# jeffersonfparil/poolgen

Hardware: NVIDIA B200
Metric: loci/sec for ols_iter (f64) (higher is better)
Workload: dtype f64

## Files before the change

poolgen_b200/csrc/pg_api.cu:

```cuda
#include <math.h>
#include <stdarg.h>
#include <stdio.h>
#include <stdlib.h>
#include <string.h>

#include <algorithm>
#include <new>

#include "pg_internal.h"
#include "pg_ptable.h"

namespace pg {
cudaError_t launch_scan_a2(const ScanParams &, int, cudaStream_t);
cudaError_t launch_scan_a3(const ScanParams &, int, cudaStream_t);
cudaError_t launch_scan_a4(const ScanParams &, int, cudaStream_t);
cudaError_t launch_scan_a5(const ScanParams &, int, cudaStream_t);
cudaError_t launch_scan_a6(const ScanParams &, int, cudaStream_t);

cudaError_t launch_scan(const ScanParams &p, int sm_count, cudaStream_t s) {
    switch (p.lay.A) {
        case 2: return launch_scan_a2(p, sm_count, s);
        case 3: return launch_scan_a3(p, sm_count, s);
        case 4: return launch_scan_a4(p, sm_count, s);
        case 5: return launch_scan_a5(p, sm_count, s);
// ... 460 lines not shown
        int rc = text_stage_a(b, b->text_src, b->text_bytes, (size_t)at + 1);
        if (rc) return rc;
        L = pg::text_parse_finish(&b->text, b->stream, &ce, &at);
    }
    if (L < 0) return pg::text_parse_fail(ctx, "upload_sync_text", L, ce, at, s->n, b->cap);
    b->n_loci = L;
    if (n_loci_out) *n_loci_out = L;
    if (L > 0 && is_regression(s))
        PG_CUDA(ctx, pg::launch_ingest_u32((const uint32_t *)b->d_stage.get(), L, s->n, s->A_in, s->drop_col, s->lay,
                                           ingest_out(b, 0), b->stream));
    return PG_OK;
}

int pg_batch_upload_sync_text(pg_batch *b, const char *text, size_t n_bytes, int64_t *n_loci_out) {
    if (n_loci_out) *n_loci_out = 0;
    int rc = text_stage_a(b, text, n_bytes, 0);
    if (rc) return rc;
    rc = text_stage_b(b, n_loci_out);
    if (rc) return rc;
    PG_CUDA(b->scan->ctx, cudaStreamSynchronize(b->stream));
    return PG_OK;
}

int pg_batch_text_labels(pg_batch *b, const uint64_t **line_offsets, const uint64_t **positions) {
    if (!b) return PG_ERR_ARG;
    if (!b->text.parsed) return fail(b->scan->ctx, PG_ERR_STATE, "pg_batch_text_labels before pg_batch_upload_sync_text");
    if (line_offsets) *line_offsets = b->text.h_out_offset.get();
    if (positions) *positions = b->text.h_out_pos.get();
    return PG_OK;
}

int pg_batch_synth(pg_batch *b, uint64_t seed, int64_t first_locus, int64_t n_loci) {
    if (!b) return PG_ERR_ARG;
    pg_scan *s = b->scan;
    pg_ctx *ctx = s->ctx;
    if (n_loci < 0 || n_loci > b->cap) return fail(ctx, PG_ERR_ARG, "synth: %lld loci > capacity %lld", (long long)n_loci, (long long)b->cap);
    PG_CUDA(ctx, cudaSetDevice(ctx->device));
    b->n_loci = n_loci;
    b->have_input = 1;
    if (n_loci == 0) return PG_OK;
    const size_t per_locus = (size_t)s->A_in * s->n * 4;
    if (!is_regression(s)) {
        int rc = ensure_stage(b, (size_t)b->cap * per_locus);
        if (rc) return rc;
        PG_CUDA(ctx, pg::launch_synth(seed, first_locus, n_loci, s->n, s->A_in, (uint32_t *)b->d_stage.get(), b->stream));
        b->input_is_counts = 1;
        return PG_OK;
    }
    int64_t slice = (int64_t)((size_t)256 << 20) / (int64_t)per_locus;
    if (slice < 1) slice = 1;
    if (slice > n_loci) slice = n_loci;
    if (b->d_stage.capacity() < (size_t)slice * per_locus) {
        int rc = ensure_stage(b, (size_t)slice * per_locus);
        if (rc) return rc;
    } else {
        slice = (int64_t)(b->d_stage.capacity() / per_locus);
        if (slice > n_loci) slice = n_loci;
    }
    for (int64_t l0 = 0; l0 < n_loci; l0 += slice) {
        const int64_t m = (n_loci - l0 < slice) ? n_loci - l0 : slice;
        PG_CUDA(ctx, pg::launch_synth(seed, first_locus + l0, m, s->n, s->A_in, (uint32_t *)b->d_stage.get(), b->stream));
        PG_CUDA(ctx, pg::launch_ingest_u32((const uint32_t *)b->d_stage.get(), m, s->n, s->A_in, s->drop_col, s->lay,
                                           ingest_out(b, l0), b->stream));
    }
    b->input_is_counts = 1;
    return PG_OK;
}

static int run_once(pg_batch *b, int *launches) {
    pg_scan *s = b->scan;
    pg_ctx *ctx = s->ctx;
    if (!b->have_input) return fail(ctx, PG_ERR_STATE, "pg_batch_run: no input uploaded");
    if (b->n_loci == 0) return PG_OK;
    if (is_regression(s)) {
        int kpass = pg::max_phen_per_pass(s->A_dev);
        {
            const int fit = (int)((size_t)(96 * 1024) / ((size_t)s->lay.n_pad * 8)) - (s->weighted ? 1 : 0);
            if (kpass > fit) kpass = fit < 1 ? 1 : fit;
        }
        static const int nbuf_env = getenv("PG_NBUF") ? atoi(getenv("PG_NBUF")) : 0;
        static const int warps_env = getenv("PG_WARPS") ? atoi(getenv("PG_WARPS")) : 0;
        static const int g_env = getenv("PG_G") ? atoi(getenv("PG_G")) : 0;
        static const int p_env = getenv("PG_P") ? atoi(getenv("PG_P")) : 0;
        if (is_nm(s)) kpass = 1;
        for (int base = 0; base < (is_nm(s) ? 1 : s->k); base += kpass) {
            pg::ScanParams p;
            memset(&p, 0, sizeof p);
            p.lay = s->lay;
            p.freq = b->d_freq.get();
            p.depth = b->d_depth.get();
            p.dmin = b->d_dmin.get();
            p.hint = b->d_hint.get();
            p.n_loci = b->n_loci;
            p.kind = is_nm(s) ? PG_KIND_OLS : s->kind;
            p.filter_only = is_nm(s) ? 1 : 0;
            p.weighted = s->weighted;
            p.maf = s->maf;
            p.one_minus_maf = 1.00 - s->maf;
            p.max_miss = s->max_miss;
            p.min_depth_f = (double)s->min_depth;
            p.w_uniform = s->w_uniform;
            p.df = s->df;
            p.inv_df = 1.0 / s->df;
            p.inv_n = 1.0 / (double)s->n;
            p.inv_nm2 = 1.0 / ((double)s->n - 2.0);
            p.ln_beta = s->ln_beta;
            p.ptab = s->d_ptab.get();
            p.ptab_isd = s->ptab_isd;
            p.ptab_bits = s->ptab_bits;
            p.ptab_t1 = s->ptab_t1;
            p.ptab_t0 = s->ptab_t0;
            p.ptab_M = s->ptab_M;
            p.K = std::min(kpass, s->k - base);
            p.y_has_nan = s->y_has_nan;
            p.yc = s->d_yc.get() + (size_t)base * s->lay.n_pad;
            p.w = s->d_w.get();
            for (int j = 0; j < p.K; j++) {
                p.ysum[j] = s->ysum[base + j];
                p.syy[j] = s->syy[base + j];
                p.ymean[j] = s->ymean[base + j];
            }
            for (int j = 0; j < s->A_dev; j++) p.codes[j] = s->codes_dev[j];
            p.meta = b->d_meta.get();
            p.freq_mean = b->d_fmean.get();
            p.stats = b->d_stats.get();
            p.defer_list = b->d_defer.get();
            p.defer_count = reinterpret_cast<uint32_t *>(b->d_defer.get() + b->cap);
            p.k_total = s->k;
            p.phen_base = base;
            p.write_meta = base == 0;
            p.nbuf_override = nbuf_env;
            p.warps_override = warps_env;
            p.g_override = g_env;
            p.p_override = p_env;
            PG_CUDA(ctx, pg::launch_scan(p, ctx->sm_count, b->stream));
            if (launches) (*launches) += 2;
        }
        if (is_nm(s)) {
            pg::NmParams q;
            memset(&q, 0, sizeof q);
            q.lay = s->lay;
            q.freq = b->d_freq.get();
            q.depth = b->d_depth.get();
            q.n_loci = b->n_loci;
            q.kind = s->kind;
            q.k = s->k;
            q.yraw = s->d_yraw.get();
            q.gw_sig = s->gw_sig;
            q.gw_min = s->gw_min;
            q.gw_max = s->gw_max;
            q.df = s->df;
            q.ln_beta = s->ln_beta;
            q.ptab = s->d_ptab.get();
            q.ptab_isd = s->ptab_isd;
            q.ptab_bits = s->ptab_bits;
            q.ptab_t1 = s->ptab_t1;
            q.ptab_t0 = s->ptab_t0;
            q.ptab_M = s->ptab_M;
            for (int j = 0; j < s->A_dev; j++) q.codes[j] = s->codes_dev[j];
            q.meta = b->d_meta.get();
            q.stats = b->d_stats.get();
            PG_CUDA(ctx, pg::launch_nm(q, ctx->sm_count, b->stream));
            if (launches) (*launches)++;
        }
    } else {
        pg::TableParams p;
        memset(&p, 0, sizeof p);
        p.counts = (const uint32_t *)b->d_stage.get();
        p.n_loci = b->n_loci;
        p.n = s->n;
        p.A_in = s->A_in;
        p.kind = s->kind;
        p.drop_col = s->drop_col;
        p.maf = s->maf;
        p.one_minus_maf = 1.00 - s->maf;
        p.max_miss = s->max_miss;
        p.min_depth_f = (double)s->min_depth;
        p.w = s->d_w.get();
// ... 187 lines not shown
```

poolgen_b200/csrc/pg_ingest.cu:

```cuda
#include <stdlib.h>

#include "pg_device.cuh"
#include "pg_internal.h"

namespace pg {

struct HintParams {
    double maf, one_minus_maf, min_depth_f;
    int enabled;
};
__device__ __forceinline__ unsigned ambiguous_alleles(const double *q, int A, int n, const HintParams &hp) {
    const double tol_rel = 4.0 * ((double)n + 8.0) * kEps;
    unsigned amb = 0;
    for (int j = 0; j < A; j++) {
        const double tl = tol_rel * fmax(fabs(q[j]), 1.0);
        if (fabs(q[j] - hp.maf) <= tl || fabs(q[j] - hp.one_minus_maf) <= tl) amb |= 1u << j;
    }
    return amb;
}

__device__ __forceinline__ uint8_t locus_hint(const double *q, int A, int n, uint32_t dm, const HintParams &hp,
                                              unsigned exact) {
    if (!hp.enabled) return 0;
    const double tol_rel = 4.0 * ((double)n + 8.0) * kEps;
    unsigned kept = 0;
    bool removed_with_reads = false, safe = true;
    for (int j = 0; j < A; j++) {
        const double tl = tol_rel * fmax(fabs(q[j]), 1.0);
        if (!((exact >> j) & 1u) && (fabs(q[j] - hp.maf) <= tl || fabs(q[j] - hp.one_minus_maf) <= tl)) safe = false;
        if (!((q[j] < hp.maf) | (q[j] > hp.one_minus_maf)))
            kept |= 1u << j;
        else if (q[j] > 0.0)
            removed_with_reads = true;
    }
    const bool depth_ok = dm != 0u && !((double)dm < hp.min_depth_f);
    return (safe && depth_ok && removed_with_reads && __popc(kept) >= 2) ? (uint8_t)(0x80u | kept) : (uint8_t)0;
}

template <typename RowFn>
__device__ __forceinline__ void ingest_loci(int64_t n_loci, const Layout &lay, int P, const double *freq,
                                            const double *__restrict__ w, uint32_t *__restrict__ dmin,
                                            uint8_t *__restrict__ hint, const HintParams &hp, RowFn &&row) {
    const int lane = threadIdx.x & 31, sub = lane / P, q0 = lane % P, lpw = 32 / P;
    const int64_t gw = ((int64_t)blockIdx.x * blockDim.x + threadIdx.x) >> 5;
    const int64_t nw = ((int64_t)gridDim.x * blockDim.x) >> 5;
    for (int64_t l0 = gw * lpw; l0 < n_loci; l0 += nw * lpw) {
        const int64_t locus = l0 + sub;
        double q[PG_MAX_ALLELES] = {0, 0, 0, 0, 0, 0};
        uint32_t dm = 0xFFFFFFFFu;
        if (locus < n_loci)
            for (int i = q0; i < lay.n_pad; i += P) row(locus, i, q, dm);
        for (int off = P >> 1; off >= 1; off >>= 1) {
            for (int j = 0; j < lay.A; j++) q[j] += __shfl_xor_sync(0xFFFFFFFFu, q[j], off);
            dm = min(dm, __shfl_xor_sync(0xFFFFFFFFu, dm, off));
        }
        unsigned amb = (hp.enabled && locus < n_loci && dm != 0u) ? ambiguous_alleles(q, lay.A, lay.n, hp) : 0u;
        if (__any_sync(0xFFFFFFFFu, amb != 0u)) {
            __syncwarp();
            const double *fl = freq + (size_t)(locus < n_loci ? locus : 0) * lay.freq_stride();
            for (int j = 0; j < lay.A; j++) {
                if (!__any_sync(0xFFFFFFFFu, (amb >> j) & 1u)) continue;
                double e = 0.0;
                for (int r0 = 0; r0 < lay.n; r0 += P) {
                    const int i = r0 + q0;
                    double term = 0.0;
                    if (i < lay.n && locus < n_loci) {
                        const double f = __ldcg(fl + lay.freq_off(i, j));
                        term = (f != f) ? 0.0 : __dmul_rn(f, w[i]);
                    }
                    const int m = min(P, lay.n - r0);
                    for (int t = 0; t < m; t++) e = __dadd_rn(e, __shfl_sync(0xFFFFFFFFu, term, t, P));
                }
                if ((amb >> j) & 1u) q[j] = e;
            }
        }
        if (locus < n_loci && q0 == 0) {
            dmin[locus] = dm;
            hint[locus] = locus_hint(q, lay.A, lay.n, dm, hp, amb);
        }
    }
}

template <typename CT>
__global__ void __launch_bounds__(256) ingest_counts_kernel(const CT *__restrict__ counts, int64_t n_loci, int n,
                                                            int A_in, int drop_col, Layout lay, int P,
                                                            double *__restrict__ freq, uint32_t *__restrict__ depth,
                                                            uint32_t *__restrict__ dmin, uint8_t *__restrict__ hint,
                                                            const double *__restrict__ w, HintParams hp) {
    ingest_loci(n_loci, lay, P, freq, w, dmin, hint, hp, [&](int64_t locus, int i, double *q, uint32_t &dm) {
        double *fl = freq + (size_t)locus * lay.freq_stride();
        if (i >= n) {
            for (int j = 0; j < lay.A; j++) fl[lay.freq_off(i, j)] = 0.0;
            depth[(size_t)locus * lay.n_pad + i] = 0xFFFFFFFFu;
            return;
        }
        const CT *cl = counts + (size_t)locus * A_in * n + i;
        uint32_t c[PG_MAX_ALLELES];
        uint64_t d = 0;
        int jj = 0;
        for (int j = 0; j < A_in; j++) {
            if (j == drop_col) continue;
            c[jj] = (uint32_t)cl[(size_t)j * n];
            d += c[jj];
            jj++;
        }
        if (d > 0xFFFFFFFEull) d = 0xFFFFFFFEull;
        const double dd = (double)d, wi = w[i];
        const double rd = __drcp_rn(dd);
        for (int j = 0; j < lay.A; j++) {
            const double cj = (double)c[j];
            const double q0 = __dmul_rn(cj, rd);
            const double f = (d == 0) ? nan("") : __fma_rn(__fma_rn(-q0, dd, cj), rd, q0);
            fl[lay.freq_off(i, j)] = f;
            if (d != 0) q[j] = fma(f, wi, q[j]);
        }
        depth[(size_t)locus * lay.n_pad + i] = (uint32_t)d;
        dm = min(dm, (uint32_t)d);
    });
}
// ... 106 lines not shown
```

poolgen_b200/csrc/pg_internal.h:

```cpp
#pragma once
#include <cuda_runtime.h>
#include <stdint.h>
#include <string>
#include <utility>
#include <vector>

#include "poolgen_cuda.h"
#include "pg_synth.h"

namespace pg {

__host__ __device__ constexpr int chunk_rows(int A) { return A <= 2 ? 256 : (A == 3 ? 192 : 128); }

struct Layout {
    int n;
    int n_pad;
    int A;
    int rc;
    int n_chunks;
    int rc_last;
    __host__ __device__ size_t freq_stride() const { return (size_t)A * n_pad; }
    __host__ __device__ size_t depth_stride() const { return (size_t)n_pad; }
    __host__ __device__ size_t freq_off(int i, int j) const {
        int c = i / rc, r = i - c * rc;
        int rcc = (c == n_chunks - 1) ? rc_last : rc;
        return (size_t)c * A * rc + (size_t)j * rcc + r;
    }
};

inline Layout make_layout(int n, int A) {
    Layout l;
    l.n = n;
    l.n_pad = (n + 3) & ~3;
    l.A = A;
    const int cr = chunk_rows(A);
    if (l.n_pad <= cr) {
        l.rc = l.n_pad;
        l.n_chunks = 1;
        l.rc_last = l.n_pad;
    } else {
        l.rc = cr;
        l.n_chunks = (l.n_pad + cr - 1) / cr;
        l.rc_last = l.n_pad - (l.n_chunks - 1) * cr;
    }
    return l;
}

constexpr int kMaxPhenPerPass = 4;
inline int max_phen_per_pass(int A) { return A <= 4 ? 4 : (A == 5 ? 3 : 2); }

struct ScanParams {
    Layout lay;
    const double *freq;
    const uint32_t *depth;
    const uint32_t *dmin;
    const uint8_t *hint;
    int64_t n_loci;
    int kind;
    int weighted;
    double maf, one_minus_maf, max_miss;
    double min_depth_f;
    double w_uniform;
    double df;
    double inv_df;
    double inv_n, inv_nm2;
    double ln_beta;
    const void *ptab;
    double ptab_isd, ptab_bits, ptab_t1, ptab_t0;
    int ptab_M;
    const double *yc;
    const double *w;
    double ysum[kMaxPhenPerPass];
    double syy[kMaxPhenPerPass];
    double ymean[kMaxPhenPerPass];
    int y_has_nan;
    int filter_only;
    uint8_t codes[8];
    uint64_t *meta;
    double *freq_mean;
    double *stats;
    uint64_t *defer_list;
    uint32_t *defer_count;
    int k_total, phen_base, K;
    int write_meta;
    uint32_t common_bytes, warp_bytes, stage_bytes;
    int nbuf, block_loci;
    int nbuf_override, warps_override, g_override, p_override;
};

struct TableParams {
    const uint32_t *counts;
    int64_t n_loci;
    int n, A_in;
    int kind;
    int drop_col;
    double maf, one_minus_maf, max_miss, min_depth_f;
    const double *w;
    uint8_t codes[8];
    uint64_t *meta;
    double *stats;
};

struct NmParams {
    Layout lay;
    const double *freq;
    const uint32_t *depth;
    int64_t n_loci;
    int kind;
    int k;
    const double *yraw;
    double gw_sig, gw_min, gw_max;
    double df, ln_beta;
    const void *ptab;
    double ptab_isd, ptab_bits, ptab_t1, ptab_t0;
    int ptab_M;
    uint8_t codes[8];
    uint64_t *meta;
    double *stats;
};
cudaError_t launch_nm(const NmParams &p, int sm_count, cudaStream_t s);

constexpr int kKinMleMaxM = 13;
struct KinMleParams {
    const double *G;
    int64_t P;
    int n, ldg, m, k;
    const double *Z;
    const double *fix;
    double df, ln_beta;
    const void *ptab;
    double ptab_isd, ptab_bits, ptab_t1, ptab_t0;
    int ptab_M;
    double *beta, *var, *pval;
};
cudaError_t launch_kin_mle(const KinMleParams &p, int sm_count, cudaStream_t s);

cudaError_t launch_scan(const ScanParams &p, int sm_count, cudaStream_t s);
cudaError_t launch_tables(const TableParams &p, int sm_count, cudaStream_t s);
struct IngestOut {
    double *freq;
    uint32_t *depth;
    uint32_t *dmin;
    uint8_t *hint;
    const double *w;
    double maf, one_minus_maf, min_depth_f;
};
cudaError_t launch_ingest_u32(const uint32_t *counts, int64_t n_loci, int n, int A_in, int drop_col, const Layout &lay,
                              const IngestOut &o, cudaStream_t s);
cudaError_t launch_ingest_u16(const uint16_t *counts, int64_t n_loci, int n, int A_in, int drop_col, const Layout &lay,
                              const IngestOut &o, cudaStream_t s);
cudaError_t launch_ingest_u8(const uint8_t *counts, int64_t n_loci, int n, int A_in, int drop_col, const Layout &lay,
                             const IngestOut &o, cudaStream_t s);
cudaError_t launch_ingest_freq(const double *freq_in, const uint32_t *depth_in, int64_t n_loci, int n, const Layout &lay,
                               const IngestOut &o, cudaStream_t s);
cudaError_t launch_synth(uint64_t seed, int64_t first_locus, int64_t n_loci, int n, int A_in,
                         uint32_t *counts, cudaStream_t s);
cudaError_t launch_widen(const void *src, int elem_bytes, uint32_t *dst, size_t count, cudaStream_t s);

template <typename T, bool Pinned>
// ... 154 lines not shown
```

poolgen_b200/csrc/pg_scan.cuh:

```cuda
#pragma once
#include "pg_device.cuh"
#include "pg_internal.h"

namespace pg {

constexpr int kScanWarps = 12;
constexpr int kRedPitch = 33;

template <int A, int K, bool W>
struct Acc {
    static constexpr int S0 = 0;
    static constexpr int P0 = S0 + A;
    static constexpr int C0 = P0 + A * (A + 1) / 2;
    static constexpr int Q0 = C0 + A * K;
    static constexpr int N = Q0 + (W ? A : 0);
    static constexpr int NP = N | 1;
    __host__ __device__ static constexpr int tri(int j, int l) {
        return P0 + j * A - j * (j - 1) / 2 + (l - j);
    }
};

template <int A, int K, bool W, bool NANAWARE>
__device__ __forceinline__ void accum_row(double (&acc)[Acc<A, K, W>::N], const double (&f)[A], const double (&y)[K],
                                          double w) {
// ... 973 lines not shown
    for (int k = 0; k < K; k++) {
        const double ptrue = in[k] ? exp(fma(s[k], fma(s[k], fma(s[k], c23[k].y, c23[k].x), c01[k].y), c01[k].x)) : 0.0;
        const double ib = 0.5 * ptrue;
        const double cdf = t_abs[k] <= tab.t_one ? 0.5 : 1.0 - ib;
        if (need[k]) pv[k] = 2.0 * (1.0 - cdf);
    }
}

template <int A, int K, int KIND>
__device__ __noinline__ void write_records(const ScanParams &p, const PTableDev &tab, int64_t locus, int status,
                                           int m, unsigned cb, const double *tb) {
    constexpr int T2 = 2 * (A - 1) * K;
    if (p.write_meta) {
        uint64_t mv = (uint64_t)status;
        if (status == PG_LOCUS_OK) {
            mv |= (uint64_t)m << 8;
#pragma unroll
            for (int s = 0; s < A - 1; s++)
                if (s < m) mv |= (uint64_t)p.codes[slot_col(cb, s)] << (16 + 8 * s);
            if (kind_is_ols<KIND>(p) && m < 6) mv |= (uint64_t)p.codes[(cb >> 20) & 0xfu] << (16 + 8 * m);
        }
        p.meta[locus] = mv;
#pragma unroll
        for (int s = 0; s < A - 1; s++)
            p.freq_mean[(size_t)locus * (A - 1) + s] = (status == PG_LOCUS_OK && s < m) ? tb[T2 + s] : nan("");
    }
#pragma unroll 1
    for (int s = 0; s < A - 1; s++) {
        const bool valid = status == PG_LOCUS_OK && s < m;
        double o0[K], o1[K], o2[K], o3[K], ta[K];
        bool need[K];
#pragma unroll
        for (int k = 0; k < K; k++) {
            const double v0 = valid ? tb[(s * K + k) * 2 + 0] : 0.0, v1 = valid ? tb[(s * K + k) * 2 + 1] : 0.0;
            o0[k] = o1[k] = o2[k] = o3[k] = nan("");
            need[k] = false;
            ta[k] = 0.0;
            if (valid) {
                if (kind_is_ols<KIND>(p)) {
                    const double se = sqrt(v1);
                    const double tt = (fabs(v0) <= kEps) ? 0.0 : v0 * rsqrt(v1);
                    o0[k] = v0;
                    o1[k] = se;
                    o2[k] = tt;
                    if (fabs(tt) <= kEps || tt != tt) {
                        o3[k] = 1.0;
                    } else {
                        need[k] = true;
                        ta[k] = fabs(tt);
                    }
                } else {
                    const double r = v0;
                    if (r == r) {
                        const double s2 = (1.0 - r * r) * p.inv_nm2;
                        o1[k] = r;
                        if (s2 <= 0.0) {
                            o0[k] = r;
                            o3[k] = kEps;
                        } else {
                            const double tt = r * rsqrt(s2);
                            o2[k] = tt;
                            o0[k] = round(r * 1e7) / 1e7;
                            if (p.lay.n > 2) {
                                need[k] = true;
                                ta[k] = fabs(tt);
                            }
                        }
                    }
                }
            }
        }
        student_batch<K>(p, tab, ta, need, o3);
#pragma unroll
        for (int k = 0; k < K; k++) {
            double *o = p.stats + (((size_t)locus * (A - 1) + s) * p.k_total + p.phen_base + k) * 4;
            *reinterpret_cast<double2 *>(o) = make_double2(o0[k], o1[k]);
            *reinterpret_cast<double2 *>(o + 2) = make_double2(o2[k], o3[k]);
        }
    }
}

template <int A, int K, bool W, bool DEFER, int KIND>
__device__ __noinline__ void epilogue(const ScanParams &p, int64_t locus, bool act, double *tot, const double *ys,
                                      const double *ws, int lane, unsigned dm, unsigned pre_kept) {
    using AC = Acc<A, K, W>;
    const PTableDev ptab = {reinterpret_cast<const double4 *>(p.ptab), p.ptab_isd, p.ptab_bits, p.ptab_t1, p.ptab_t0, p.ptab_M};
    double *tg = tot + (size_t)lane * AC::NP;
    const double tol_rel = 2.0 * ((double)p.lay.n + 8.0) * kEps;
    int status = PG_LOCUS_FILTERED;
    unsigned kept = 0, exact_bits = 0;
    bool slow = false, slow_decide = false;
    double q[A];
#pragma unroll
    for (int j = 0; j < A; j++) q[j] = 0.0;
    bool deferred = false, kept_known = false;
    if (act && pre_kept) {
        status = PG_LOCUS_OK;
        kept = pre_kept;
        if (DEFER) {
            kept_known = true;
#pragma unroll
            for (int j = 0; j < A; j++)
                if (((kept >> j) & 1u) && tg[AC::S0 + j] != tg[AC::S0 + j]) deferred = true;
        }
    } else if (act) {
        if ((double)dm < p.min_depth_f) {
            status = PG_LOCUS_FILTERED;
        } else if (dm == 0u) {
            status = PG_LOCUS_OK;
            slow = slow_decide = true;
        } else {
            status = PG_LOCUS_OK;
#pragma unroll
            for (int j = 0; j < A; j++) {
                q[j] = W ? tg[AC::Q0 + j] : tg[AC::S0 + j] * p.w_uniform;
                const double tl = tol_rel * fmax(fabs(q[j]), 1.0);
                if (fabs(q[j] - p.maf) <= tl || fabs(q[j] - p.one_minus_maf) <= tl) exact_bits |= 1u << j;
            }
        }
    }
    if (DEFER) {
        if (exact_bits != 0u) deferred = true;
    } else {
        unsigned need = __ballot_sync(PG_FULL_MASK, exact_bits != 0u);
        while (need) {
            const int src = __ffs(need) - 1;
            need &= need - 1;
            const unsigned bits = __shfl_sync(PG_FULL_MASK, exact_bits, src);
            const int64_t lsrc = __shfl_sync(PG_FULL_MASK, locus, src);
#pragma unroll
            for (int j = 0; j < A; j++) {
                if (!((bits >> j) & 1u)) continue;
                const double v = exact_q(p, lsrc, j, ws, lane);
                if (lane == src) q[j] = v;
            }
        }
    }
    if (act && status == PG_LOCUS_OK && !slow && !deferred && !pre_kept) {
#pragma unroll
        for (int j = 0; j < A; j++)
            if (!((q[j] < p.maf) | (q[j] > p.one_minus_maf))) kept |= 1u << j;
        if (__popc(kept) < 2) {
            status = PG_LOCUS_FILTERED;
        } else {
#pragma unroll
            for (int j = 0; j < A; j++)
                if (!((kept >> j) & 1u) && tg[AC::S0 + j] > 0.0) slow = true;
        }
    }
    if (DEFER) {
        if (act && slow && status == PG_LOCUS_OK) {
            kept_known = !deferred && !slow_decide;
            deferred = true;
        }
    } else {
        unsigned need = __ballot_sync(PG_FULL_MASK, act && slow && status == PG_LOCUS_OK);
        while (need) {
            const int src = __ffs(need) - 1;
            need &= need - 1;
            const bool dec = __shfl_sync(PG_FULL_MASK, (int)slow_decide, src) != 0;
            unsigned kk = __shfl_sync(PG_FULL_MASK, kept, src);
            const int64_t lsrc = __shfl_sync(PG_FULL_MASK, locus, src);
            const int st = slow_locus<A, K, W>(p, lsrc, ys, ws, tot + (size_t)src * AC::NP, lane, dec, kk);
            if (lane == src) {
                status = st;
                kept = kk;
            }
        }
        __syncwarp();
    }
    int m = 0, redo_mode = REDO_NONE;
    unsigned cb = 0;
    if (act && status == PG_LOCUS_OK && !deferred)
        solve_locus<A, K, W, DEFER, KIND>(p, locus, tg, status, kept, m, cb, redo_mode);
    if (DEFER) {
        uint64_t why = (exact_bits != 0u ? 1u : 0u) | ((slow && !slow_decide) ? 2u : 0u) | (slow_decide ? 4u : 0u) |
                       ((deferred && pre_kept) ? 8u : 0u);
        if (redo_mode != REDO_NONE) {
            deferred = true;
            why |= (uint64_t)redo_mode << 4;
        }
        if (deferred)
            p.defer_list[atomicAdd(p.defer_count, 1u)] =
                (uint64_t)locus | (kept_known ? ((uint64_t)kept << 40) : 0ull) | (why << 56);
    } else {
        unsigned need = __ballot_sync(PG_FULL_MASK, redo_mode != REDO_NONE);
        while (need) {
            const int src = __ffs(need) - 1;
            need &= need - 1;
            const int md = __shfl_sync(PG_FULL_MASK, redo_mode, src);
            const unsigned kk = __shfl_sync(PG_FULL_MASK, kept, src);
            const int mm = __shfl_sync(PG_FULL_MASK, m, src);
            const unsigned cc = __shfl_sync(PG_FULL_MASK, cb, src);
            const int64_t lsrc = __shfl_sync(PG_FULL_MASK, locus, src);
            __syncwarp();
            const int st = (md == REDO_CORR_NAN)
                               ? corr_pairwise_locus<A, K>(p, lsrc, kk, mm, cc, ys, tot + (size_t)src * AC::NP, lane)
                           : (md == REDO_MINNORM)
                               ? minnorm_locus<A, K>(p, lsrc, kk, mm, cc, ys, tot + (size_t)src * AC::NP, lane)
                               : redo_locus<A, K>(p, lsrc, kk, mm, cc, md, ys, tot + (size_t)src * AC::NP, lane);
            if (lane == src) status = st;
        }
        __syncwarp();
    }
    if (act && !deferred) write_records<A, K, KIND>(p, ptab, locus, status, m, cb, tg);
    __syncwarp();
}

constexpr int kFixWarps = 8;

template <int A, int K, bool W>
__global__ void __launch_bounds__(kFixWarps * 32) fixup_kernel(const __grid_constant__ ScanParams p) {
    using AC = Acc<A, K, W>;
    extern __shared__ __align__(16) unsigned char fsm[];
    __shared__ __align__(16) ScanParams sp_storage;
    for (int i = threadIdx.x; i < (int)(sizeof(ScanParams) / 4); i += blockDim.x)
        reinterpret_cast<uint32_t *>(&sp_storage)[i] = reinterpret_cast<const uint32_t *>(&p)[i];
    __syncthreads();
    const ScanParams &sp = sp_storage;
    const int warp = threadIdx.x >> 5, lane = threadIdx.x & 31;
    const uint32_t count = *p.defer_count;
    const int n_pad = p.lay.n_pad;
    const double *ys = p.yc;
    const double *ws = W ? p.w : nullptr;
    const uint32_t per_blk = min(32u, max(1u, (count + gridDim.x - 1) / gridDim.x));
    const uint32_t n_blocks = (count + per_blk - 1) / per_blk;
    int it = 0;
    for (uint32_t blk = blockIdx.x; blk < n_blocks; blk += gridDim.x, it++) {
        double *tot = reinterpret_cast<double *>(fsm) + (size_t)(it & 1) * 32 * AC::NP;
        const uint32_t e0 = blk * per_blk;
        const int cnt = (int)min(per_blk, count - e0);
        for (int g = warp; g < cnt; g += kFixWarps) {
            const uint64_t e = p.defer_list[e0 + g];
            const int64_t locus = (int64_t)(e & 0xFFFFFFFFFFull);
            const unsigned kept = (unsigned)(e >> 40) & 0x3fu;
            double acc[AC::N];
#pragma unroll
            for (int a = 0; a < AC::N; a++) acc[a] = 0.0;
            if (kept) {
                for_rows_coop<A>(sp, locus, lane, [&](int r, const double(&f)[A], uint32_t d) {
                    double F[A], y[K];
                    renorm_row_fast<A>(f, d, kept, F);
#pragma unroll
                    for (int k = 0; k < K; k++) y[k] = ys[k * n_pad + r];
                    accum_row<A, K, W, true>(acc, F, y, 0.0);
                });
            } else {
                for_rows_coop<A>(sp, locus, lane, [&](int r, const double(&f)[A], uint32_t) {
                    double y[K];
#pragma unroll
                    for (int k = 0; k < K; k++) y[k] = ys[k * n_pad + r];
                    accum_row<A, K, W, false>(acc, f, y, W ? ws[r] : 0.0);
                });
            }
#pragma unroll
            for (int a = 0; a < AC::N; a++) {
                const double v = warp_sum_fixed(acc[a]);
                if (lane == 0) tot[(size_t)g * AC::NP + a] = v;
            }
        }
        __syncthreads();
        if (warp == (it % kFixWarps)) {
            const uint64_t mine = (lane < cnt) ? p.defer_list[e0 + lane] : 0ull;
            const int64_t locus = (int64_t)(mine & 0xFFFFFFFFFFull);
            const unsigned dm = (lane < cnt) ? __ldg(p.dmin + locus) : 0xFFFFFFFFu;
            epilogue<A, K, W, false, -1>(sp, locus, lane < cnt, tot, ys, ws, lane, dm, (unsigned)(mine >> 40) & 0x3fu);
        }
    }
}

template <int A, int K, bool W, int P, int KIND>
__global__ void __launch_bounds__(kScanWarps * 32, 1) scan_kernel(const __grid_constant__ ScanParams p) {
    using AC = Acc<A, K, W>;
    constexpr int LPS = 32 / P;
    constexpr int RC = chunk_rows(A);
    extern __shared__ __align__(128) unsigned char smem[];
    __shared__ __align__(16) ScanParams sp_storage;
    for (int i = threadIdx.x; i < (int)(sizeof(ScanParams) / 4); i += blockDim.x)
        reinterpret_cast<uint32_t *>(&sp_storage)[i] = reinterpret_cast<const uint32_t *>(&p)[i];
    const ScanParams &sp = sp_storage;
    const Layout lay = p.lay;
    const int n_pad = lay.n_pad;
    const int G = p.block_loci;
    const int warp = threadIdx.x >> 5, lane = threadIdx.x & 31, nwarps = blockDim.x >> 5;
    double *ys = reinterpret_cast<double *>(smem);
    double *ws = W ? ys + (size_t)K * n_pad : nullptr;
    unsigned char *wb = smem + p.common_bytes + (size_t)warp * p.warp_bytes;
    uint64_t *bars = reinterpret_cast<uint64_t *>(wb);
    unsigned char *stage0 = wb + 64;
    double *tot = reinterpret_cast<double *>(stage0 + (size_t)p.nbuf * p.stage_bytes);
    const int nbuf = p.nbuf;
    const int red_rows = max(1, min((int)(p.stage_bytes / (kRedPitch * 8)), AC::N));

    for (int i = threadIdx.x; i < K * n_pad; i += blockDim.x) ys[i] = p.yc[i];
    if (W)
        for (int i = threadIdx.x; i < n_pad; i += blockDim.x) ws[i] = p.w[i];
    if (lane == 0) {
        for (int b = 0; b < nbuf; b++) mbar_init(&bars[b], 1);
        fence_mbar_init();
    }
    __syncthreads();

    const int64_t L = p.n_loci;
    const int64_t NB = (L + G - 1) / G;
    const int64_t gw = (int64_t)blockIdx.x * nwarps + warp;
    const int64_t TW = (int64_t)gridDim.x * nwarps;
    if (gw >= NB) return;
    const int n_chunks = lay.n_chunks;
    const size_t fstride = lay.freq_stride();
    const uint32_t full_bytes = (uint32_t)(A * lay.rc * 8), last_bytes = (uint32_t)(A * lay.rc_last * 8);
    const uint32_t locus_bytes = (uint32_t)(fstride * 8);

    int64_t i_blk = gw;
    const unsigned char *i_src = reinterpret_cast<const unsigned char *>(p.freq + (size_t)(gw * G) * fstride);
    int i_left = (int)min((int64_t)G, L - gw * G);
    int i_chunk = 0;
    bool i_done = false;
    auto issue_next = [&](int b, bool scratch_used) {
        if (i_done) return;
        uint32_t bytes;
        int nl = 1;
        if (P == 32) {
            bytes = (i_chunk == n_chunks - 1) ? last_bytes : full_bytes;
        } else {
            nl = min(LPS, i_left);
            bytes = (uint32_t)nl * locus_bytes;
        }
        if (lane == 0) {
            if (scratch_used) fence_proxy_async();
            mbar_expect_tx(&bars[b], bytes);
            bulk_g2s(stage0 + (size_t)b * p.stage_bytes, i_src, bytes, &bars[b]);
        }
        i_src += bytes;
        if (P == 32) {
            if (++i_chunk == n_chunks) {
                i_chunk = 0;
                i_left--;
            }
        } else {
            i_left -= nl;
        }
        if (i_left == 0) {
            i_blk += TW;
            if (i_blk >= NB) {
                i_done = true;
            } else {
                i_src = reinterpret_cast<const unsigned char *>(p.freq + (size_t)(i_blk * G) * fstride);
                i_left = (int)min((int64_t)G, L - i_blk * G);
            }
        }
    };
    for (int b = 0; b < nbuf; b++) issue_next(b, false);

    int buf = 0;
    uint32_t parity = 0;
    auto load_meta = [&](int64_t b, unsigned &dm_o, unsigned &hl_o) {
        const int64_t m0 = b * G;
        const bool in = b < NB && lane < (int)min((int64_t)G, L - m0);
        dm_o = in ? __ldg(p.dmin + m0 + lane) : 0xFFFFFFFFu;
        hl_o = in ? (unsigned)__ldg(p.hint + m0 + lane) : 0u;
    };
    unsigned dm_next, hl_next;
    load_meta(gw, dm_next, hl_next);
    for (int64_t blk = gw; blk < NB; blk += TW) {
        const int64_t l0 = blk * G;
        const int cnt = (int)min((int64_t)G, L - l0);
        const unsigned dm = dm_next, hl = hl_next;
        load_meta(blk + TW, dm_next, hl_next);
        if (P == 32) {
            for (int g = 0; g < cnt; g++) {
                const unsigned hk = __shfl_sync(PG_FULL_MASK, hl, g);
                const bool hinted = (hk & 0x80u) != 0u;
                const unsigned hkept = hk & 0x3fu;
                double acc[AC::N];
#pragma unroll
                for (int i = 0; i < AC::N; i++) acc[i] = 0.0;
                for (int chunk = 0; chunk < n_chunks; chunk++) {
                    const double *yrow = ys + chunk * RC + 2 * lane;
                    const double *wrow = W ? ws + chunk * RC + 2 * lane : nullptr;
                    mbar_wait(&bars[buf], parity);
                    double *fb = reinterpret_cast<double *>(stage0 + (size_t)buf * p.stage_bytes);
                    if (chunk < n_chunks - 1 || lay.rc_last == RC) {
                        const double *fl = fb + 2 * lane;
#pragma unroll
                        for (int it = 0; it < RC / 64; it++) {
                            double2 f2[A], y2[K];
#pragma unroll
                            for (int j = 0; j < A; j++) f2[j] = *reinterpret_cast<const double2 *>(fl + j * RC + it * 64);
#pragma unroll
                            for (int k = 0; k < K; k++)
                                y2[k] = *reinterpret_cast<const double2 *>(yrow + (size_t)k * n_pad + it * 64);
                            double2 w2 = make_double2(0.0, 0.0);
                            if (W) w2 = *reinterpret_cast<const double2 *>(wrow + it * 64);
                            if (hinted) renorm_pair<A>(f2, hkept, chunk * RC + it * 64 + 2 * lane, lay.n);
                            accum_pair<A, K, W>(acc, f2, y2, w2);
                        }
                    } else {
                        const int rcc = lay.rc_last;
                        for (int r = 2 * lane; r < rcc; r += 64) {
                            double2 f2[A], y2[K];
#pragma unroll
                            for (int j = 0; j < A; j++) f2[j] = *reinterpret_cast<const double2 *>(fb + (size_t)j * rcc + r);
#pragma unroll
                            for (int k = 0; k < K; k++)
                                y2[k] = *reinterpret_cast<const double2 *>(ys + chunk * RC + (size_t)k * n_pad + r);
                            double2 w2 = make_double2(0.0, 0.0);
                            if (W) w2 = *reinterpret_cast<const double2 *>(ws + chunk * RC + r);
                            if (hinted) renorm_pair<A>(f2, hkept, chunk * RC + r, lay.n);
                            accum_pair<A, K, W>(acc, f2, y2, w2);
                        }
                    }
                    __syncwarp();
                    if (chunk == n_chunks - 1)
                        reduce_to_tot<AC::N, AC::NP, 32>(acc, fb, red_rows, tot + (size_t)g * AC::NP, lane);
                    issue_next(buf, chunk == n_chunks - 1);
                    if (++buf == nbuf) {
                        buf = 0;
                        parity ^= 1u;
                    }
                }
            }
        } else {
            const int u = lane / P, q0 = lane % P;
            const int nsteps = (cnt + LPS - 1) / LPS;
            for (int s = 0; s < nsteps; s++) {
                double acc[AC::N];
#pragma unroll
                for (int i = 0; i < AC::N; i++) acc[i] = 0.0;
                const unsigned hk = __shfl_sync(PG_FULL_MASK, hl, min(s * LPS + u, 31));
                const bool hinted = (hk & 0x80u) != 0u;
                const unsigned hkept = hk & 0x3fu;
                mbar_wait(&bars[buf], parity);
                double *fb = reinterpret_cast<double *>(stage0 + (size_t)buf * p.stage_bytes);
                const double *fl = fb + (size_t)u * fstride;
                if (__any_sync(PG_FULL_MASK, hinted)) {
                    if (s * LPS + u < cnt) {
#pragma unroll 1
                        for (int r = 2 * q0; r < n_pad; r += 2 * P) {
                            double2 f2[A], y2[K];
#pragma unroll
                            for (int j = 0; j < A; j++)
                                f2[j] = *reinterpret_cast<const double2 *>(fl + (size_t)j * n_pad + r);
#pragma unroll
                            for (int k = 0; k < K; k++)
                                y2[k] = *reinterpret_cast<const double2 *>(ys + (size_t)k * n_pad + r);
                            double2 w2 = make_double2(0.0, 0.0);
                            if (W) w2 = *reinterpret_cast<const double2 *>(ws + r);
                            if (hinted) renorm_pair<A>(f2, hkept, r, lay.n);
                            accum_pair<A, K, W>(acc, f2, y2, w2);
                        }
                    }
                } else if (s * LPS + u < cnt) {
#pragma unroll 2
                    for (int r = 2 * q0; r < n_pad; r += 2 * P) {
                        double2 f2[A], y2[K];
#pragma unroll
                        for (int j = 0; j < A; j++) f2[j] = *reinterpret_cast<const double2 *>(fl + (size_t)j * n_pad + r);
#pragma unroll
                        for (int k = 0; k < K; k++) y2[k] = *reinterpret_cast<const double2 *>(ys + (size_t)k * n_pad + r);
                        double2 w2 = make_double2(0.0, 0.0);
                        if (W) w2 = *reinterpret_cast<const double2 *>(ws + r);
                        accum_pair<A, K, W>(acc, f2, y2, w2);
                    }
                }
                __syncwarp();
                reduce_to_tot<AC::N, AC::NP, P>(acc, fb, red_rows, tot + (size_t)(s * LPS) * AC::NP, lane);
                issue_next(buf, true);
                if (++buf == nbuf) {
                    buf = 0;
                    parity ^= 1u;
                }
            }
        }
        epilogue<A, K, W, true, KIND>(sp, l0 + lane, lane < cnt, tot, ys, ws, lane, dm, (hl & 0x80u) ? (hl & 0x3fu) : 0u);
    }
}

template <int A, int K, bool W, int P>
cudaError_t launch_scan_p(ScanParams p, int sm_count, cudaStream_t s) {
    using AC = Acc<A, K, W>;
    const Layout &lay = p.lay;
    const size_t avail = 227 * 1024 - 512;
    size_t common = (size_t)(K + (W ? 1 : 0)) * lay.n_pad * 8;
    common = (common + 127) / 128 * 128;
    size_t stage = (P == 32) ? (size_t)A * lay.rc * 8 : (size_t)(32 / P) * lay.freq_stride() * 8;
    stage = (stage + 127) / 128 * 128;
    if (stage < (size_t)kRedPitch * 8) stage = ((size_t)kRedPitch * 8 + 127) / 128 * 128;
    int G = 32, nbuf = 3, nwarps = 0;
    size_t wbytes = 0;
    auto fit = [&](int g, int nb) {
        const size_t tot_bytes = ((size_t)g * AC::NP * 8 + 127) / 128 * 128;
        wbytes = 64 + (size_t)nb * stage + tot_bytes;
        nwarps = common + wbytes <= avail ? (int)((avail - common) / wbytes) : 0;
        if (nwarps > kScanWarps) nwarps = kScanWarps;
        return nwarps;
    };
    const int g_min = (P == 32) ? 16 : 32;
    if (p.nbuf_override >= 1 || p.g_override >= 1) {
        G = (p.g_override == 16 || p.g_override == 32) && P == 32 ? p.g_override : 32;
        nbuf = (p.nbuf_override >= 1 && p.nbuf_override <= 8) ? p.nbuf_override : 2;
        fit(G, nbuf);
    } else if (fit(32, 3) >= kScanWarps) {
        G = 32, nbuf = 3;
    } else if (fit(32, 2) >= kScanWarps) {
        G = 32, nbuf = 2;
    } else if (fit(g_min, 2) >= kScanWarps) {
        G = g_min, nbuf = 2;
    } else {
        G = 32, nbuf = 2;
        fit(G, nbuf);
    }
    if (p.warps_override >= 1 && p.warps_override < nwarps) nwarps = p.warps_override;
    if (nwarps < 1) return cudaErrorInvalidConfiguration;
    if (p.g_override < 1 && p.n_loci > 0) {
        const int64_t gw = (int64_t)sm_count * nwarps;
        const int step = (P == 32) ? 1 : 32 / P;
        const int64_t r = (p.n_loci + gw * G - 1) / (gw * G);
        int64_t g = (p.n_loci + gw * r - 1) / (gw * r);
        g = (g + step - 1) / step * step;
        if (g < step) g = step;
        if (g < G) G = (int)g;
    }
    p.common_bytes = (uint32_t)common;
    p.warp_bytes = (uint32_t)wbytes;
    p.stage_bytes = (uint32_t)stage;
    p.nbuf = nbuf;
    p.block_loci = G;
    const size_t smem = common + (size_t)nwarps * wbytes;
    auto kern = (p.kind == PG_KIND_OLS) ? scan_kernel<A, K, W, P, PG_KIND_OLS> : scan_kernel<A, K, W, P, PG_KIND_CORR>;
    cudaError_t e = cudaFuncSetAttribute(kern, cudaFuncAttributeMaxDynamicSharedMemorySize, (int)smem);
    if (e != cudaSuccess) return e;
    const int64_t NB = (p.n_loci + G - 1) / G;
    int64_t ctas = (NB + nwarps - 1) / nwarps;
    if (ctas > sm_count) ctas = sm_count;
    if (ctas < 1) ctas = 1;
    e = cudaMemsetAsync(p.defer_count, 0, 4, s);
    if (e != cudaSuccess) return e;
    kern<<<(unsigned)ctas, nwarps * 32, smem, s>>>(p);
    e = cudaGetLastError();
    if (e != cudaSuccess) return e;
    auto fix = fixup_kernel<A, K, W>;
    const size_t fsmem = (size_t)2 * 32 * AC::NP * 8;
    e = cudaFuncSetAttribute(fix, cudaFuncAttributeMaxDynamicSharedMemorySize, (int)fsmem);
    if (e != cudaSuccess) return e;
    fix<<<sm_count * 8, kFixWarps * 32, fsmem, s>>>(p);
    return cudaGetLastError();
}

template <int A, int K, bool W>
cudaError_t launch_scan_t(const ScanParams &p, int sm_count, cudaStream_t s) {
    if (p.lay.n_chunks == 1) {
        const int P = p.p_override ? p.p_override : (p.lay.n_pad > 64 ? 16 : 8);
        if (P == 16) return launch_scan_p<A, K, W, 16>(p, sm_count, s);
        return launch_scan_p<A, K, W, 8>(p, sm_count, s);
    }
    return launch_scan_p<A, K, W, 32>(p, sm_count, s);
}
// ... 19 lines not shown
```

Before: 215.4 million.

## Skip TMA loads and accumulation for loci already filtered by depth or hint

```diff
diff --git a/poolgen_b200/csrc/pg_api.cu b/poolgen_b200/csrc/pg_api.cu
--- a/poolgen_b200/csrc/pg_api.cu
+++ b/poolgen_b200/csrc/pg_api.cu
@@ -566,6 +566,7 @@
         static const int warps_env = getenv("PG_WARPS") ? atoi(getenv("PG_WARPS")) : 0;
         static const int g_env = getenv("PG_G") ? atoi(getenv("PG_G")) : 0;
         static const int p_env = getenv("PG_P") ? atoi(getenv("PG_P")) : 0;
+        static const bool no_skip = getenv("PG_NOSKIP") != nullptr;
         if (is_nm(s)) kpass = 1;
         for (int base = 0; base < (is_nm(s) ? 1 : s->k); base += kpass) {
             pg::ScanParams p;
@@ -578,6 +579,7 @@
             p.n_loci = b->n_loci;
             p.kind = is_nm(s) ? PG_KIND_OLS : s->kind;
             p.filter_only = is_nm(s) ? 1 : 0;
+            p.skip = no_skip ? 0 : 1;
             p.weighted = s->weighted;
             p.maf = s->maf;
             p.one_minus_maf = 1.00 - s->maf;
diff --git a/poolgen_b200/csrc/pg_ingest.cu b/poolgen_b200/csrc/pg_ingest.cu
--- a/poolgen_b200/csrc/pg_ingest.cu
+++ b/poolgen_b200/csrc/pg_ingest.cu
@@ -34,7 +34,9 @@
             removed_with_reads = true;
     }
     const bool depth_ok = dm != 0u && !((double)dm < hp.min_depth_f);
-    return (safe && depth_ok && removed_with_reads && __popc(kept) >= 2) ? (uint8_t)(0x80u | kept) : (uint8_t)0;
+    if (!safe || !depth_ok) return 0;
+    if (__popc(kept) < 2) return 0x40;
+    return removed_with_reads ? (uint8_t)(0x80u | kept) : (uint8_t)0;
 }
 
 template <typename RowFn>
diff --git a/poolgen_b200/csrc/pg_internal.h b/poolgen_b200/csrc/pg_internal.h
--- a/poolgen_b200/csrc/pg_internal.h
+++ b/poolgen_b200/csrc/pg_internal.h
@@ -75,6 +75,7 @@
     double ymean[kMaxPhenPerPass];
     int y_has_nan;
     int filter_only;
+    int skip;
     uint8_t codes[8];
     uint64_t *meta;
     double *freq_mean;
diff --git a/poolgen_b200/csrc/pg_scan.cuh b/poolgen_b200/csrc/pg_scan.cuh
--- a/poolgen_b200/csrc/pg_scan.cuh
+++ b/poolgen_b200/csrc/pg_scan.cuh
@@ -1079,7 +1079,7 @@
 
 template <int A, int K, bool W, bool DEFER, int KIND>
 __device__ __noinline__ void epilogue(const ScanParams &p, int64_t locus, bool act, double *tot, const double *ys,
-                                      const double *ws, int lane, unsigned dm, unsigned pre_kept) {
+                                      const double *ws, int lane, unsigned dm, unsigned pre_kept, bool skipped) {
     using AC = Acc<A, K, W>;
     const PTableDev ptab = {reinterpret_cast<const double4 *>(p.ptab), p.ptab_isd, p.ptab_bits, p.ptab_t1, p.ptab_t0, p.ptab_M};
     double *tg = tot + (size_t)lane * AC::NP;
@@ -1101,7 +1101,7 @@
                 if (((kept >> j) & 1u) && tg[AC::S0 + j] != tg[AC::S0 + j]) deferred = true;
         }
     } else if (act) {
-        if ((double)dm < p.min_depth_f) {
+        if (skipped || (double)dm < p.min_depth_f) {
             status = PG_LOCUS_FILTERED;
         } else if (dm == 0u) {
             status = PG_LOCUS_OK;
@@ -1261,7 +1261,8 @@
             const uint64_t mine = (lane < cnt) ? p.defer_list[e0 + lane] : 0ull;
             const int64_t locus = (int64_t)(mine & 0xFFFFFFFFFFull);
             const unsigned dm = (lane < cnt) ? __ldg(p.dmin + locus) : 0xFFFFFFFFu;
-            epilogue<A, K, W, false, -1>(sp, locus, lane < cnt, tot, ys, ws, lane, dm, (unsigned)(mine >> 40) & 0x3fu);
+            epilogue<A, K, W, false, -1>(sp, locus, lane < cnt, tot, ys, ws, lane, dm, (unsigned)(mine >> 40) & 0x3fu,
+                                         false);
         }
     }
 }
@@ -1299,20 +1300,49 @@
     __syncthreads();
 
     const int64_t L = p.n_loci;
-    const int64_t NB = (L + G - 1) / G;
     const int64_t gw = (int64_t)blockIdx.x * nwarps + warp;
     const int64_t TW = (int64_t)gridDim.x * nwarps;
-    if (gw >= NB) return;
+    const int64_t r_first = gw * G;
+    auto round_base = [&](int64_t r) { return r_first + r * TW * G; };
+    auto round_cnt = [&](int64_t base) { return base < L ? (int)min((int64_t)G, L - base) : 0; };
+    if (r_first >= L) return;
     const int n_chunks = lay.n_chunks;
     const size_t fstride = lay.freq_stride();
     const uint32_t full_bytes = (uint32_t)(A * lay.rc * 8), last_bytes = (uint32_t)(A * lay.rc_last * 8);
     const uint32_t locus_bytes = (uint32_t)(fstride * 8);
-
-    int64_t i_blk = gw;
-    const unsigned char *i_src = reinterpret_cast<const unsigned char *>(p.freq + (size_t)(gw * G) * fstride);
-    int i_left = (int)min((int64_t)G, L - gw * G);
+    auto locus_src = [&](int64_t locus) { return reinterpret_cast<const unsigned char *>(p.freq + (size_t)locus * fstride); };
+
+    auto load_meta = [&](int64_t r, unsigned &dm_o, unsigned &hl_o) {
+        const int64_t m0 = round_base(r);
+        const bool in = lane < round_cnt(m0);
+        dm_o = in ? __ldg(p.dmin + m0 + lane) : 0xFFFFFFFFu;
+        hl_o = in ? (unsigned)__ldg(p.hint + m0 + lane) : 0u;
+    };
+    auto live_mask = [&](int cnt, unsigned dm, unsigned hl) {
+        const bool skip = p.skip && (((double)dm < p.min_depth_f) || (hl & 0x40u) != 0u);
+        return __ballot_sync(PG_FULL_MASK, lane < cnt && !skip);
+    };
+
+    int64_t i_r = 0;
+    const unsigned char *i_src = locus_src(r_first);
+    int i_left = round_cnt(r_first);
+    unsigned i_live = 0;
+    unsigned i_dm = 0, i_hl = 0;
     int i_chunk = 0;
     bool i_done = false;
+    auto seek_live = [&]() {
+        while (i_live == 0u) {
+            const int c = round_cnt(round_base(++i_r));
+            if (c == 0) {
+                i_done = true;
+                return;
+            }
+            const unsigned dm = i_dm, hl = i_hl;
+            load_meta(i_r + 1, i_dm, i_hl);
+            i_live = live_mask(c, dm, hl);
+        }
+        i_src = locus_src(round_base(i_r) + __ffs(i_live) - 1);
+    };
     auto issue_next = [&](int b, bool scratch_used) {
         if (i_done) return;
         uint32_t bytes;
@@ -1332,40 +1362,44 @@
         if (P == 32) {
             if (++i_chunk == n_chunks) {
                 i_chunk = 0;
-                i_left--;
+                i_live &= i_live - 1u;
+                seek_live();
             }
         } else {
             i_left -= nl;
-        }
-        if (i_left == 0) {
-            i_blk += TW;
-            if (i_blk >= NB) {
-                i_done = true;
-            } else {
-                i_src = reinterpret_cast<const unsigned char *>(p.freq + (size_t)(i_blk * G) * fstride);
-                i_left = (int)min((int64_t)G, L - i_blk * G);
+            if (i_left == 0) {
+                const int64_t base = round_base(++i_r);
+                i_left = round_cnt(base);
+                if (i_left == 0)
+                    i_done = true;
+                else
+                    i_src = locus_src(base);
             }
         }
     };
+
+    unsigned dm_next, hl_next;
+    load_meta(0, dm_next, hl_next);
+    if (P == 32) {
+        load_meta(1, i_dm, i_hl);
+        i_live = live_mask(i_left, dm_next, hl_next);
+        seek_live();
+    }
     for (int b = 0; b < nbuf; b++) issue_next(b, false);
 
     int buf = 0;
     uint32_t parity = 0;
-    auto load_meta = [&](int64_t b, unsigned &dm_o, unsigned &hl_o) {
-        const int64_t m0 = b * G;
-        const bool in = b < NB && lane < (int)min((int64_t)G, L - m0);
-        dm_o = in ? __ldg(p.dmin + m0 + lane) : 0xFFFFFFFFu;
-        hl_o = in ? (unsigned)__ldg(p.hint + m0 + lane) : 0u;
-    };
-    unsigned dm_next, hl_next;
-    load_meta(gw, dm_next, hl_next);
-    for (int64_t blk = gw; blk < NB; blk += TW) {
-        const int64_t l0 = blk * G;
-        const int cnt = (int)min((int64_t)G, L - l0);
+    for (int64_t rnd = 0;; rnd++) {
+        const int64_t l0 = round_base(rnd);
+        const int cnt = round_cnt(l0);
+        if (cnt == 0) break;
         const unsigned dm = dm_next, hl = hl_next;
-        load_meta(blk + TW, dm_next, hl_next);
+        load_meta(rnd + 1, dm_next, hl_next);
+        unsigned live = 0;
         if (P == 32) {
-            for (int g = 0; g < cnt; g++) {
+            live = live_mask(cnt, dm, hl);
+            for (unsigned todo = live; todo; todo &= todo - 1u) {
+                const int g = __ffs(todo) - 1;
                 const unsigned hk = __shfl_sync(PG_FULL_MASK, hl, g);
                 const bool hinted = (hk & 0x80u) != 0u;
                 const unsigned hkept = hk & 0x3fu;
@@ -1469,7 +1503,8 @@
                 }
             }
         }
-        epilogue<A, K, W, true, KIND>(sp, l0 + lane, lane < cnt, tot, ys, ws, lane, dm, (hl & 0x80u) ? (hl & 0x3fu) : 0u);
+        epilogue<A, K, W, true, KIND>(sp, l0 + lane, lane < cnt, tot, ys, ws, lane, dm,
+                                      (hl & 0x80u) ? (hl & 0x3fu) : 0u, P == 32 && lane < cnt && !((live >> lane) & 1u));
     }
 }
 
```

New measurement: 228.5 million, median of 6. 6.1% higher.
